# UnofficialJuliaMirrorSnapshots/TrajectoryOptimization.jl-c79d492b-0548-5874-b488-5a62c1d9d0ca

Hardware: AMD Instinct MI355X
Metric: iLQR iterations/sec (batched trajectories), quadrotor n=13 m=4 N=101 (higher is better)
Workload: dtype f64

## Files before the change

### trajectoryoptimization.jl-c79d492b-0548-5874-b488-5a62c1d9d0ca_amd/csrc/tog_host_plan.hpp

```cpp
#pragma once
#include <algorithm>
#include <cmath>
#include <cstddef>
#include <cstring>
#include <type_traits>
#include <vector>

namespace tog_plan {

template <int... Vs, class F>
inline void pick(int v, F&& f) {
  (void)((v == Vs && (f(std::integral_constant<int, Vs>{}), true)) || ...);
}

inline bool chol_upper(const double* A, int n, double* U) {
  for (int i = 0; i < n * n; i++) U[i] = 0.0;
  for (int j = 0; j < n; j++) {
    double s = A[j + n * j];
    for (int k = 0; k < j; k++) s -= U[k + n * j] * U[k + n * j];
    if (!(s > 0.0)) return false;
    const double ujj = std::sqrt(s);
    U[j + n * j] = ujj;
    for (int c = j + 1; c < n; c++) {
      double t = A[j + n * c];
      for (int k = 0; k < j; k++) t -= U[k + n * j] * U[k + n * c];
      U[j + n * c] = t / ujj;
    }
  }
  return true;
}

struct CostPlan {
  int nc_in = 0, kst = 0, nk = 0;
  int n = 0, m = 0;
  std::vector<double> kc;
  std::vector<double> cQf;
  bool sqrt_ok = false;
  int diag_cost = 0;
  const double* Q(int k) const { return kc.data() + (size_t)k * kst; }
  const double* R(int k) const { return Q(k) + n * n; }
  const double* H(int k) const { return R(k) + m * m; }
  const double* q(int k) const { return H(k) + m * n; }
  const double* r(int k) const { return q(k) + n; }
  double c(int k) const { return Q(k)[nc_in - 1]; }
  const double* cQ(int k) const { return Q(k) + nc_in; }
  const double* cR(int k) const { return cQ(k) + n * n; }
};

inline CostPlan plan_costs(int n, int m, int N, double dt, const double* Q, const double* R, const double* H,
                           const double* q, const double* r, double c, const double* stage_costs,
                           const double* Qf) {
  CostPlan p;
  p.n = n;
  p.m = m;
  p.nc_in = n * n + m * m + m * n + n + m + 1;
  p.kst = 2 * n * n + 2 * m * m + m * n + n + m + 1;
  p.nk = stage_costs ? N - 1 : 1;
  const int nc_in = p.nc_in, nk = p.nk;
  p.kc.assign((size_t)nk * p.kst, 0.0);
  for (int k = 0; k < nk; k++) {
    double* o = p.kc.data() + (size_t)k * p.kst;
    if (stage_costs) {
      memcpy(o, stage_costs + (size_t)k * nc_in, sizeof(double) * nc_in);
    } else {
      memcpy(o, Q, sizeof(double) * n * n);
      memcpy(o + n * n, R, sizeof(double) * m * m);
      memcpy(o + n * n + m * m, H, sizeof(double) * m * n);
      memcpy(o + n * n + m * m + m * n, q, sizeof(double) * n);
      memcpy(o + n * n + m * m + m * n + n, r, sizeof(double) * m);
      o[nc_in - 1] = c;
    }
  }
  auto kcQ = [&](int k) { return p.kc.data() + (size_t)k * p.kst + nc_in; };
  auto kcR = [&](int k) { return kcQ(k) + n * n; };
  p.cQf.assign((size_t)n * n, 0.0);
  bool ok = chol_upper(Qf, n, p.cQf.data());
  std::vector<double> Qdt((size_t)n * n), Rdt((size_t)m * m);
  for (int k = 0; k < nk; k++) {
    for (int i = 0; i < n * n; i++) Qdt[i] = p.Q(k)[i] * dt;
    for (int i = 0; i < m * m; i++) Rdt[i] = p.R(k)[i] * dt;
    ok = chol_upper(Qdt.data(), n, kcQ(k)) && chol_upper(Rdt.data(), m, kcR(k)) && ok;
  }
  p.sqrt_ok = ok;
  bool diag = true;
  for (int j = 0; j < n; j++)
    for (int i = 0; i < n; i++)
      if (i != j && Qf[i + n * j] != 0.0) diag = false;
  for (int k = 0; k < nk; k++) {
    for (int j = 0; j < n; j++)
      for (int i = 0; i < n; i++)
        if (i != j && p.Q(k)[i + n * j] != 0.0) diag = false;
    for (int j = 0; j < m; j++)
      for (int i = 0; i < m; i++)
        if (i != j && p.R(k)[i + m * j] != 0.0) diag = false;
    for (int i = 0; i < m * n; i++)
// ... 44 lines not shown
```

### trajectoryoptimization.jl-c79d492b-0548-5874-b488-5a62c1d9d0ca_amd/csrc/tog_kernels.hpp

```cpp
#pragma once

#include "tog_device.hpp"
#include <string.h>

namespace tog {

constexpr int PCAP = 72;
template <class M>
__host__ __device__ constexpr int pcap_of() { return PCAP; }
constexpr int WAVE = 64;

__device__ __forceinline__ long long traj_of_slot(const DevBuffers& Bf, long long i, long long B) {
  if (Bf.act_list) return i < (long long)*Bf.act_count ? (long long)Bf.act_list[i] : -1;
  return i < B ? i : -1;
}
__device__ __forceinline__ long long slot_count(const DevBuffers& Bf, long long B) {
  return Bf.act_list ? (long long)*Bf.act_count : B;
}

__device__ __forceinline__ void wsync() { __syncthreads(); }

template <class M>
__host__ __device__ constexpr int cand_w() {
  return M::n + M::m;
// ... 2482 lines not shown
  const long long b = (phase == 2) ? (long long)list[t] : traj_of_slot(Bf, t, P->B);
  if (!Bf.st[b].active) return;
  if (phase == 1 && !ls_decided_within(P->o, Bf, b, Bf.nc, bookkeeping ? Bf.st[b].J : Jprev_in[b], Bf.st[b].dV0,
                                       Bf.st[b].dV1, hi))
    return;
  constexpr int n = M::n, m = M::m;
  const tog_options& o = P->o;
  const bool al = (mode == TOG_MODE_AL);
  const int N = P->N, NC = Bf.nc;
  TrajState s = Bf.st[b];
  const double J_prev = bookkeeping ? s.J : Jprev_in[b];
  double J = INFINITY, z = -1.0, expected = 0.0, alpha_last = 0.0;
  int trials = 0, state = 0;
  for (int jj = 0;; jj++) {
    if (!((z <= o.line_search_lower_bound || z > o.line_search_upper_bound) && J >= J_prev)) {
      state = 1;
      break;
    }
    if (jj > o.iterations_linesearch) {
      state = 2;
      break;
    }
    trials++;
    const double aj = ldexp(1.0, -jj);
    bool ok;
    double Jj;
    if (jj < NC) {
      ok = Bf.lsok[b * NC + jj] != 0;
      Jj = Bf.lsJ[b * NC + jj];
    } else {
      ok = rollout_cost<M, INTEG, 0>(P, Bf, b, aj, al, Jj, nullptr, RT);
    }
    if (!ok) continue;
    J = Jj;
    expected = -aj * (s.dV0 + aj * s.dV1);
    z = (expected > 0.0) ? (J_prev - J) / expected : -1.0;
    alpha_last = aj;
  }
  double grad = 0.0;
  bool copied = false;
  if (state == 2) {
    const double* X = Bf.X + (size_t)b * N * n;
    const double* U = Bf.U + (size_t)b * (N - 1) * m;
    if (!bookkeeping) {
      double* Xb = Bf.Xb + (size_t)b * N * n;
      double* Ub = Bf.Ub + (size_t)b * (N - 1) * m;
      for (int i = 0; i < N * n; i++) Xb[i] = X[i];
      for (int i = 0; i < (N - 1) * m; i++) Ub[i] = U[i];
    }
    J = traj_cost<M>(P, Bf, b, X, U, al, al ? Bf.C + (size_t)b * N * P->pmax : nullptr);
    z = 0.0;
    expected = 0.0;
    alpha_last = 0.0;
    reg_increase(P, s);
    s.rho += o.bp_reg_fp;
    grad = traj_gradient<M>(P, Bf, b, al);
    copied = true;
  } else if (!bookkeeping) {
    double Jw;
    rollout_cost<M, INTEG, 1>(P, Bf, b, alpha_last, al, Jw, nullptr, RT);
  } else if (!(J > o.max_cost_value)) {
    double Jw;
    rollout_cost<M, INTEG, 2>(P, Bf, b, alpha_last, al, Jw, &grad, RT);
    copied = true;
  }
  if (bookkeeping && copied && state != 2 && o.gradient_type != 0) grad = traj_gradient<M>(P, Bf, b, al);
  s.alpha = alpha_last;
  s.z = z;
  s.expected = expected;
  s.ls_trials = trials;
  if (J > J_prev) s.flags |= TOG_TRAJ_COST_INCREASED;
  if (Jout) Jout[b] = J;
  if (bookkeeping) {
    if (s.flags & TOG_TRAJ_COST_INCREASED) {
      s.active = 0;
    } else {
      step_bookkeeping<M>(P, Bf, b, s, J, copied, grad, mode);
    }
  }
  Bf.st[b] = s;
}


template <class M>
__global__ void __launch_bounds__(256) k_ls_decide(const DevProblem* __restrict__ P, DevBuffers Bf, int hi,
                                                   int bookkeeping, const double* __restrict__ Jprev_in,
                                                   const int* __restrict__ in_list, const int* __restrict__ in_count,
                                                   int* __restrict__ out_list, int* __restrict__ out_count, int pend) {
  const long long t = (long long)blockIdx.x * blockDim.x + threadIdx.x;
  const long long nb = in_list ? (long long)*in_count : slot_count(Bf, P->B);
  bool und = false;
  long long b = 0;
  if (t < nb) {
    b = in_list ? (long long)in_list[t] : traj_of_slot(Bf, t, P->B);
    TrajState* st = Bf.st + b;
    if (st->active) {
      const tog_options& o = P->o;
      const int NC = Bf.nc;
      const double J_prev = bookkeeping ? st->J : Jprev_in[b];
      const double dV0 = st->dV0, dV1 = st->dV1;
      if (pend) hi = (st->ls_pend + hi < NC) ? st->ls_pend + hi : NC;
      double J = INFINITY, z = -1.0, expected = 0.0, alpha_last = 0.0;
      int trials = 0, state = 0, win = -1;
      for (int jj = 0;; jj++) {
        if (!((z <= o.line_search_lower_bound || z > o.line_search_upper_bound) && J >= J_prev)) {
          state = 1;
          break;
        }
        if (jj > o.iterations_linesearch) {
          state = 2;
          break;
        }
        if (jj >= hi) break;
        trials++;
        if (!Bf.lsok[b * NC + jj]) continue;
        const double aj = ldexp(1.0, -jj);
        J = Bf.lsJ[b * NC + jj];
        expected = -aj * (dV0 + aj * dV1);
        z = (expected > 0.0) ? (J_prev - J) / expected : -1.0;
        alpha_last = aj;
        win = jj;
      }
      if (state == 0) {
        und = true;
        if (pend) {
          st->ls_pend = hi;
          Bf.ls_win[b] = -9;
        }
      } else {
        st->ls_pend = 0;
        if (state == 2) {
          win = -2;
          z = 0.0;
          expected = 0.0;
          alpha_last = 0.0;
          if (Bf.ls_fb) Bf.ls_fb[atomicAdd(Bf.ls_count + 2, 1)] = (int)b;
        } else if (win < 0) {
          win = -3;
        }
        st->alpha = alpha_last;
        st->z = z;
        st->expected = expected;
        st->ls_trials = trials;
        Bf.ls_win[b] = win;
        Bf.ls_Jw[b] = J;
      }
    }
  }
  if (!out_list || pend) return;
  const unsigned long long mask = __ballot(und);
  if (mask == 0) return;
  const int lane = threadIdx.x & (WAVE - 1);
  const int leader = __ffsll((long long)mask) - 1;
  int base = 0;
  if (lane == leader) base = atomicAdd(out_count, __popcll(mask));
  base = __shfl(base, leader);
  if (und) out_list[base + __popcll(mask & ((1ull << lane) - 1))] = (int)b;
}

template <class M>
__global__ void __launch_bounds__(256) k_ls_apply(const DevProblem* __restrict__ P, DevBuffers Bf, int bookkeeping) {
  constexpr int n = M::n, m = M::m, Q = cand_q<M>();
  const int N = P->N;
  const unsigned per = (unsigned)N * Q;
  const unsigned long long t = (unsigned long long)blockIdx.x * blockDim.x + threadIdx.x;
  const long long slot = (long long)(t / per);
  if (slot >= slot_count(Bf, P->B)) return;
  const long long b = traj_of_slot(Bf, slot, P->B);
  const unsigned r = (unsigned)(t - (unsigned long long)slot * per);
  const int k = (int)(r / Q), q = (int)(r - (unsigned)k * Q);
  if (!Bf.st[b].active) return;
  const int w = Bf.ls_win[b];
  if (w < 0) return;
  if (bookkeeping && Bf.ls_Jw[b] > P->o.max_cost_value) return;
  const int ncp = Bf.ncp;
  const double* tb = Bf.cand + (size_t)b * per * ncp * 4;
  const double* src = tb + ((size_t)r * ncp + w) * 4;
  double v[4];
#pragma unroll
  for (int e = 0; e < 4; e++) v[e] = src[e];
  double* Xd = (bookkeeping ? Bf.X : Bf.Xb) + ((size_t)b * N + k) * n;
  double* Ud = (bookkeeping ? Bf.U : Bf.Ub) + ((size_t)b * (N - 1) + k) * m;
#pragma unroll
  for (int e = 0; e < 4; e++) {
    const int c = 4 * q + e;
    if (c < m) {
      if (k < N - 1) Ud[c] = v[e];
    } else if (c < m + n) {
      Xd[c - m] = (k == 0) ? Bf.x0[(size_t)b * n + c - m] : v[e];
    }
  }
  if (bookkeeping && q == 0 && k < N - 1) {
    const double* dk = Bf.d + ((size_t)b * (N - 1) + k) * m;
    double mx = -INFINITY;
#pragma unroll
    for (int i = 0; i < m; i++) {
      const double ui = (i < 4) ? v[i] : tb[cand_at(k, i, Q, ncp) + (size_t)w * 4];
      const double vv = fabs(dk[i]) / (fabs(ui) + 1.0);
      if (vv > mx || isnan(vv)) mx = vv;
    }
    Bf.gk[(size_t)b * N + k] = mx;
  }
}

template <class M, int INTEG>
__device__ __noinline__ void replay_cost(const DevProblem* __restrict__ P, const DevBuffers& Bf, long long b,
                                         double alpha, bool al, int bookkeeping, double max_cost, double J,
                                         double& grad, bool& copied, const RowTables& RT) {
  double Jw;
  if (!bookkeeping) {
    rollout_cost<M, INTEG, 1>(P, Bf, b, alpha, al, Jw, nullptr, RT);
  } else if (!(J > max_cost)) {
    rollout_cost<M, INTEG, 2>(P, Bf, b, alpha, al, Jw, &grad, RT);
    copied = true;
  }
}

template <class M>
__global__ void __launch_bounds__(64) k_ls_fallback(const DevProblem* __restrict__ P, DevBuffers Bf, int al,
                                                    const int* __restrict__ list, const int* __restrict__ count) {
  if ((int)blockIdx.x >= *count) return;
  extern __shared__ double fb_lds[];
  constexpr int n = M::n, m = M::m;
  const int N = P->N, pmax = P->pmax;
  const long long b = list[blockIdx.x];
  const int lane = threadIdx.x;
  double* sk = fb_lds;
  double* ak = fb_lds + N;
  int* hk = reinterpret_cast<int*>(fb_lds + 2 * N);
  const double* X = Bf.X + (size_t)b * N * n;
  const double* U = Bf.U + (size_t)b * (N - 1) * m;
  const double* d = Bf.d + (size_t)b * (N - 1) * m;
  double* C = Bf.C + (size_t)b * N * pmax;
  const double* lam = Bf.lam + (size_t)b * N * pmax;
  const double* mu = Bf.mu + (size_t)b * N * pmax;
  for (int k = lane; k < N; k += WAVE) {
    const double* x = X + (size_t)k * n;
    const double* u = (k < N - 1) ? U + (size_t)k * m : nullptr;
    sk[k] = (k < N - 1) ? stage_cost_m<M>(P, b, k, x, u) : terminal_cost_m<M>(P, b, x);
    const int cnt = al ? knot_count(P, k) : 0;
    const cptr<ConRow> rows = knot_rows(P, k);
    double lc = 0.0, cIc = 0.0;
    for (int i = 0; i < cnt; i++) {
      const size_t q = (size_t)k * pmax + i;
      const ConRow r = traj_row(P, b, load_row(rows + i));
      const double c = row_value_m<M>(r, x, u);
      const double l = lam[q];
      const bool a = row_inequality<(ModelTraits<M>::slack > 0)>(r) ? ((c >= 0.0) || (l > 0.0)) : true;
      const double w = a ? mu[q] : 0.0;
      lc = fma(l, c, lc);
      cIc = fma(c * w, c, cIc);
      C[q] = c;
    }
    ak[k] = lc + 0.5 * cIc;
    hk[k] = cnt;
    if (k < N - 1) {
      double mx = -INFINITY;
#pragma unroll
      for (int i = 0; i < m; i++) {
        const double v = fabs(d[(size_t)k * m + i]) / (fabs(u[i]) + 1.0);
        if (v > mx || isnan(v)) mx = v;
      }
      Bf.gk[(size_t)b * N + k] = mx;
    }
  }
  __syncthreads();
  if (lane != 0) return;
  double J = 0.0, Jc = 0.0;
  for (int k = 0; k < N - 1; k++) J += sk[k];
  J += sk[N - 1];
  for (int k = 0; k < N; k++)
    if (hk[k]) Jc += ak[k];
  Bf.ls_Jw[b] = al ? J + Jc : J;
}

template <class M, int INTEG>
__global__ void __launch_bounds__(64) k_ls_book(const DevProblem* __restrict__ P, DevBuffers Bf, int mode,
                                                int bookkeeping, const double* Jprev_in, double* Jout) {
  const long long t = (long long)blockIdx.x * blockDim.x + threadIdx.x;
  extern __shared__ double rt_lds[];
  const RowTables RT =
      (mode == TOG_MODE_AL && Bf.rows_lds > 0) ? block_row_tables(P, rt_lds) : global_row_tables(P);
  if (t >= slot_count(Bf, P->B)) return;
  const long long b = traj_of_slot(Bf, t, P->B);
  if (!Bf.st[b].active) return;
  constexpr int n = M::n, m = M::m;
  const tog_options& o = P->o;
  const bool al = (mode == TOG_MODE_AL);
  const int N = P->N;
  const int win = Bf.ls_win[b];
  if (win == -9) return;
  TrajState s = Bf.st[b];
  double J = Bf.ls_Jw[b];
  const double J_prev = bookkeeping ? s.J : Jprev_in[b];
  double grad = 0.0;
  bool copied = false;
  if (win == -2) {
    if (!bookkeeping) {
      const double* X = Bf.X + (size_t)b * N * n;
      const double* U = Bf.U + (size_t)b * (N - 1) * m;
      double* Xb = Bf.Xb + (size_t)b * N * n;
      double* Ub = Bf.Ub + (size_t)b * (N - 1) * m;
      for (int i = 0; i < N * n; i++) Xb[i] = X[i];
      for (int i = 0; i < (N - 1) * m; i++) Ub[i] = U[i];
    }
    reg_increase(P, s);
    s.rho += o.bp_reg_fp;
    if (o.gradient_type == 0) {
      const double* g = Bf.gk + (size_t)b * N;
      double gsum = 0.0;
      for (int k = 0; k < N - 1; k++) gsum += g[k];
      grad = gsum / N;
    } else {
      grad = traj_gradient<M>(P, Bf, b, al);
    }
    copied = true;
  } else if (win == -3) {
    replay_cost<M, INTEG>(P, Bf, b, s.alpha, al, bookkeeping, o.max_cost_value, J, grad, copied, RT);
  } else if (bookkeeping && !(J > o.max_cost_value)) {
    const double* g = Bf.gk + (size_t)b * N;
    double gsum = 0.0;
    for (int k = 0; k < N - 1; k++) gsum += g[k];
    grad = gsum / N;
    copied = true;
  }
  if (bookkeeping && copied && win != -2 && o.gradient_type != 0) grad = traj_gradient<M>(P, Bf, b, al);
  if (J > J_prev) s.flags |= TOG_TRAJ_COST_INCREASED;
  if (Jout) Jout[b] = J;
  (void)copied;
  if (bookkeeping) {
    if (s.flags & TOG_TRAJ_COST_INCREASED) {
      s.active = 0;
    } else if (inner_bookkeeping(P, Bf, b, s, J, grad, mode)) {
      Bf.ls_done[atomicAdd(Bf.ls_count + 1, 1)] = (int)b;
    }
  }
  Bf.st[b] = s;
}

template <class M>
__global__ void __launch_bounds__(64) k_al_outer(const DevProblem* __restrict__ P, DevBuffers Bf, int mode,
                                                 const int* __restrict__ list, const int* __restrict__ count) {
  if ((int)blockIdx.x >= *count) return;
  extern __shared__ double alo_lds[];
  constexpr int n = M::n, m = M::m;
  constexpr bool SL = ModelTraits<M>::slack > 0;
  const int N = P->N, pmax = P->pmax;
  const tog_options& o = P->o;
  const long long b = list[blockIdx.x];
  const int lane = threadIdx.x;
  double* sk = alo_lds;
  double* ak = alo_lds + N;
  int* hk = reinterpret_cast<int*>(alo_lds + 2 * N);
  const double* X = Bf.X + (size_t)b * N * n;
  const double* U = Bf.U + (size_t)b * (N - 1) * m;
  double* C = Bf.C + (size_t)b * N * pmax;
  double* lam = Bf.lam + (size_t)b * N * pmax;
  double* mu = Bf.mu + (size_t)b * N * pmax;
  double mumax = 0.0, cmax = 0.0;
  for (int k = lane; k < N; k += WAVE) {
    const double* x = X + (size_t)k * n;
    const double* u = (k < N - 1) ? U + (size_t)k * m : nullptr;
    sk[k] = (k < N - 1) ? stage_cost_m<M>(P, b, k, x, u) : terminal_cost_m<M>(P, b, x);
    const int cnt = knot_count(P, k);
    const cptr<ConRow> rows = knot_rows(P, k);
    double lc = 0.0, cIc = 0.0, e = 0.0, im = -INFINITY;
    int ni = 0;
    for (int i = 0; i < cnt; i++) {
      const size_t q = (size_t)k * pmax + i;
      const ConRow r = traj_row(P, b, load_row(rows + i));
      const double c = row_value_m<M>(r, x, u);
      C[q] = c;
      const bool ineq = row_inequality<SL>(r);
      double l = lam[q] + mu[q] * c;
      l = tog_jlmax(o.dual_min, tog_jlmin(o.dual_max, l));
      if (ineq) l = tog_jlmax(0.0, l);
      const double mn = fmax(0.0, fmin(o.penalty_max, o.penalty_scaling * mu[q]));
      lam[q] = l;
      mu[q] = mn;
      mumax = fmax(mumax, mn);
      if (ineq) {
        ni++;
        im = tog_jlmax(im, c);
      } else {
        e = tog_jlmax(e, fabs(c));
      }
      const bool a = ineq ? ((c >= 0.0) || (l > 0.0)) : true;
      const double w = a ? mn : 0.0;
      lc = fma(l, c, lc);
      cIc = fma(c * w, c, cIc);
    }
    if (cnt) {
      cmax = tog_jlmax(e, cmax);
      if (ni > 0) cmax = tog_jlmax(tog_jlmax(0.0, im), cmax);
    }
    ak[k] = lc + 0.5 * cIc;
    hk[k] = cnt;
  }
#pragma unroll
  for (int off = 32; off >= 1; off >>= 1) {
    mumax = fmax(mumax, __shfl_xor(mumax, off));
    cmax = tog_jlmax(cmax, __shfl_xor(cmax, off));
  }
  __syncthreads();
  if (lane != 0) return;
  TrajState s = Bf.st[b];
  const bool conv = (o.kickout_max_penalty && mumax == o.penalty_max) || (cmax < o.constraint_tolerance);
  double Jnext = 0.0;
  if (!conv && s.al_iter < o.al_iterations) {
    double J = 0.0, Jc = 0.0;
    for (int k = 0; k < N - 1; k++) J += sk[k];
    J += sk[N - 1];
    for (int k = 0; k < N; k++)
      if (hk[k]) Jc += ak[k];
    Jnext = J + Jc;
  }
  const double gnext = (Bf.hist_in && !conv && s.al_iter < o.al_iterations) ? traj_gradient<M>(P, Bf, b, true) : 0.0;
  al_outer_finish(P, Bf, b, s, mumax, cmax, s.J, Jnext, gnext, mode);
  Bf.st[b] = s;
}

}
#include "tog_bwd_team.hpp"
#include "tog_bwd_quad.hpp"
#include "tog_pn.hpp"
namespace tog {

template <class M, int INTEG>
__global__ void __launch_bounds__(64) k_slack_controls(const DevProblem* __restrict__ P, DevBuffers Bf) {
  using Mb = typename ModelTraits<M>::Base;
  constexpr int n = M::n, m = M::m;
  const long long b = (long long)blockIdx.x * blockDim.x + threadIdx.x;
  if (b >= P->B) return;
  const int N = P->N;
  const double* X = Bf.X + (size_t)b * N * n;
  double* U = Bf.U + (size_t)b * (N - 1) * m;
  double x[n], xn[n];
#pragma unroll
  for (int i = 0; i < n; i++) x[i] = Bf.x0[(size_t)b * n + i];
  for (int k = 0; k < N - 1; k++) {
    double* u = U + (size_t)k * m;
    discrete_step<Mb, INTEG>(xn, x, u, P->dt);
#pragma unroll
    for (int i = 0; i < n; i++) {
      const double sl = X[(size_t)(k + 1) * n + i] - xn[i];
      u[Mb::m + i] = sl;
      x[i] = xn[i] + sl;
    }
  }
}

__device__ inline bool dev_chol_upper(double* U, const double* A, int n) {
  for (int i = 0; i < n * n; i++) U[i] = 0.0;
  for (int j = 0; j < n; j++) {
    double s = A[j + n * j];
    for (int k = 0; k < j; k++) s -= U[k + n * j] * U[k + n * j];
    if (!(s > 0.0)) return false;
    const double ujj = sqrt(s);
    U[j + n * j] = ujj;
    for (int c = j + 1; c < n; c++) {
      double t = A[j + n * c];
      for (int k = 0; k < j; k++) t -= U[k + n * j] * U[k + n * c];
      U[j + n * c] = t / ujj;
    }
  }
  return true;
}

__device__ inline void dev_qr_R(double* R, double* Pm, int rows, int cols) {
  const int kmax = rows < cols ? rows : cols;
  for (int j = 0; j < kmax; j++) {
    const double alpha = Pm[j + rows * j];
    double acc[4] = {0.0, 0.0, 0.0, 0.0};
    for (int i = j + 1; i < rows; i++) acc[(i - j - 1) & 3] = fma(Pm[i + rows * j], Pm[i + rows * j], acc[(i - j - 1) & 3]);
    const double ss = (acc[0] + acc[1]) + (acc[2] + acc[3]);
    if (ss == 0.0) continue;
    const double beta = -copysign(sqrt(fma(alpha, alpha, ss)), alpha);
    const double vd = alpha - beta;
    const double rd = 1.0 / (beta * vd);
    Pm[j + rows * j] = beta;
    for (int c = j + 1; c < cols; c++) {
      double a4[4] = {0.0, 0.0, 0.0, 0.0};
      for (int i = j + 1; i < rows; i++) a4[(i - j - 1) & 3] = fma(Pm[i + rows * j], Pm[i + rows * c], a4[(i - j - 1) & 3]);
      const double p = fma(vd, Pm[j + rows * c], (a4[0] + a4[1]) + (a4[2] + a4[3])) * rd;
      Pm[j + rows * c] = fma(vd, p, Pm[j + rows * c]);
      for (int i = j + 1; i < rows; i++) Pm[i + rows * c] = fma(Pm[i + rows * j], p, Pm[i + rows * c]);
    }
  }
  for (int j = 0; j < cols; j++)
    for (int i = 0; i < cols; i++) R[i + cols * j] = (i <= j && i < rows) ? Pm[i + rows * j] : 0.0;
}

template <class M>
__global__ void __launch_bounds__(64) k_cost_expansion(const DevProblem* __restrict__ P, DevBuffers Bf, int sq,
                                                       int al, int* fail) {
  constexpr int n = M::n, m = M::m, NQ = nq_of<M>(), PC = pcap_of<M>(), W = n > m ? n : m;
  const long long t = (long long)blockIdx.x * blockDim.x + threadIdx.x;
  const int N = P->N;
  if (t >= P->B * (long long)N) return;
  const int k = (int)(t % N);
  const long long b = t / N;
  const bool term = (k == N - 1);
// ... 126 lines not shown
```

### trajectoryoptimization.jl-c79d492b-0548-5874-b488-5a62c1d9d0ca_amd/csrc/tog_launch.hpp

```cpp
#pragma once

#include "tog_kernels.hpp"
#include "tog_host_plan.hpp"

namespace tog {

using tog_plan::pick;

inline int ali_backward(int al, int tv) { return (al ? 1 : 0) | (tv ? 2 : 0); }
inline int ali_expand(int al, int tv) { return (al ? 1 : 0) | ((tv & 2) ? 2 : 0); }

struct StreamPair {
  hipStream_t st2;
  hipEvent_t fork, join;
};

struct ModelOps {
  int n, m;
  int slack;
  int pcap;
  int has_con;
  int min_time;
  long long jws_per_lane;
  void (*slack_controls)(const DevProblem*, const DevBuffers&, long long B, int integ, hipStream_t);
// ... 41 lines not shown
    }
    if (integ == TOG_RK4) {
      f(std::integral_constant<int, TOG_RK4>{});
    } else if (integ == TOG_MIDPOINT) {
      f(std::integral_constant<int, TOG_MIDPOINT>{});
    } else if (integ == TOG_RK3_IMPLICIT || integ == TOG_MIDPOINT_IMPLICIT) {
      if constexpr (ModelTraits<M>::implicit_ok) {
        if (integ == TOG_RK3_IMPLICIT)
          f(std::integral_constant<int, TOG_RK3_IMPLICIT>{});
        else
          f(std::integral_constant<int, TOG_MIDPOINT_IMPLICIT>{});
      }
    } else {
      f(std::integral_constant<int, TOG_RK3>{});
    }
  }
  static void init(const DevProblem* P, const DevBuffers& Bf, long long B, int integ, int mode, hipStream_t st) {
    with_integ(integ, [&](auto ic) {
      constexpr int I = decltype(ic)::value;
      hipLaunchKernelGGL((k_init<M, I>), dim3(grid(B, 64)), dim3(64), 0, st, P, Bf, mode);
    });
  }
  static void refill(const DevProblem* P, const DevBuffers& Bf, int count, int N, int integ, int mode, const int* list,
                     const double* x0, const double* U, const double* X, hipStream_t st) {
    if (count <= 0) return;
    const unsigned sm = (unsigned)(N * (2 * sizeof(double) + sizeof(int)));
    with_integ(integ, [&](auto ic) {
      constexpr int I = decltype(ic)::value;
      hipLaunchKernelGGL((k_refill<M, I>), dim3((unsigned)count), dim3(64), sm, st, P, Bf, mode, list, count, x0, U, X);
    });
  }
  static void rollout_open(const DevProblem* P, const DevBuffers& Bf, long long B, int integ, hipStream_t st) {
    with_integ(integ, [&](auto ic) {
      constexpr int I = decltype(ic)::value;
      hipLaunchKernelGGL((k_rollout_open<M, I>), dim3(grid(B, 64)), dim3(64), 0, st, P, Bf);
    });
  }
  static void jacobian(const DevProblem* P, const DevBuffers& Bf, long long B, int N, int integ, hipStream_t st) {
    if constexpr (ModelTraits<M>::min_time) {
      using Mc = typename ModelTraits<M>::Core;
      constexpr int NCHT = (Mc::n + Mc::m + 1 + JW - 1) / JW;
      const long long total = B * (long long)(N - 1) * NCHT;
      with_integ(integ, [&](auto ic) {
        constexpr int I = decltype(ic)::value;
        hipLaunchKernelGGL((k_jacobian_mt<M, I, JW>), dim3(grid(total, 256)), dim3(256), 0, st, P, Bf, total);
      });
    } else if (Mb::id == TOG_MODEL_KUKA && integ == TOG_RK3 && Bf.jws) {
      if constexpr (Mb::id == TOG_MODEL_KUKA && ModelTraits<M>::explicit_ok) {
        const long long total = B * (long long)(N - 1);
        hipLaunchKernelGGL((k_kuka_points<M>), dim3(grid(total, 64)), dim3(64), 0, st, P, Bf, total);
        hipLaunchKernelGGL((k_kuka_sjac<M, 0>), dim3(grid(total * 21, 256)), dim3(256), 0, st, P, Bf, total);
        hipLaunchKernelGGL((k_kuka_sjac<M, 1>), dim3(grid(total * 21, 256)), dim3(256), 0, st, P, Bf, total);
        hipLaunchKernelGGL((k_kuka_chain<M>), dim3((unsigned)total), dim3(64), 0, st, P, Bf, total);
      }
    } else {
      constexpr int NCH = (Mb::n + Mb::m + JW - 1) / JW;
      const long long total = B * (long long)(N - 1) * NCH;
      with_integ(integ, [&](auto ic) {
        constexpr int I = decltype(ic)::value;
        hipLaunchKernelGGL((k_jacobian<M, I, JW>), dim3(grid(total, 256)), dim3(256), 0, st, P, Bf, total);
      });
    }
  }
  static void backward(const DevProblem* P, const DevBuffers& Bf, long long B, int sq, int al, int flags, int team,
                       hipStream_t st) {
    if constexpr (M::m <= M::n && M::n + 1 <= 16 && !ModelTraits<M>::min_time) {
    if (team) {
      constexpr int TPW = TeamCfg<M>::TPW;
      const dim3 g((unsigned)((B + TPW - 1) / TPW)), blk(64);
      DevBuffers Bl = Bf;
      Bl.bwd_stride = Bf.bwd_stride2[sq ? 1 : 0];
      Bl.bwd_shmem = Bf.bwd_shmem2[sq ? 1 : 0];
      const unsigned sm = (unsigned)Bl.bwd_shmem;
      const int ali = ali_backward(al, Bf.tv);
      auto launch = [&](auto wpe_c) {
        pick<0, 1>(sq ? 1 : 0, [&](auto sq_c) {
          pick<0, 1, 2, 3>(ali, [&](auto ali_c) {
            hipLaunchKernelGGL((k_bwd_team<M, decltype(sq_c)::value, decltype(ali_c)::value, decltype(wpe_c)::value>),
                               g, blk, sm, st, P, Bl, flags);
          });
        });
      };
      const char* tk = getenv("TOG_BWD_TAIL");
      const bool quad = !(tk && !strcmp(tk, "team"));
      if (Bf.tail && sq && TeamCfg<M>::TEAM == 16 && quad) {
        if constexpr (TeamCfg<M>::TEAM == 16) {
          pick<0, 1, 2, 3>(ali, [&](auto ali_c) {
            hipLaunchKernelGGL((k_bwd_quad<M, decltype(ali_c)::value>), dim3((unsigned)B), dim3(256), 0, st, P, Bf,
                               flags);
          });
        }
      } else if (Bf.tail || (B + TPW - 1) / TPW <= Bf.simds) {
        launch(std::integral_constant<int, 1>{});
      } else {
        launch(std::integral_constant<int, TOG_BWD_WAVES>{});
      }
      return;
    }
    }
    pick<0, 1>(sq ? 1 : 0, [&](auto sq_c) {
      pick<0, 1>(al ? 1 : 0, [&](auto al_c) {
        hipLaunchKernelGGL((k_backward<M, decltype(sq_c)::value, decltype(al_c)::value>), dim3((unsigned)B), dim3(64),
                           0, st, P, Bf, flags);
      });
    });
  }
  static void expand(const DevProblem* P, const DevBuffers& Bf, long long B, int N, int pmax, int sq, int al,
                     hipStream_t st) {
    if constexpr (M::m <= M::n && M::n + 1 <= 16 && !ModelTraits<M>::min_time) {
      constexpr int TPW = TeamCfg<M>::TPW;
      const unsigned sm = (unsigned)(sizeof(double) * TPW * expand_team_stride<M>(pmax));
      int mode = 0;
      const int ali = ali_expand(al, Bf.tv);
      if constexpr (M::m <= 4 && TeamCfg<M>::TEAM == 16) {
        const char* eq = getenv("TOG_EXPAND_QUAD");
        if (sq && !(eq && eq[0] == '0')) {
          const long long qteams = B * (long long)(N - 1);
          pick<0, 1, 2, 3>(ali, [&](auto ali_c) {
            hipLaunchKernelGGL((k_expand_u<M, decltype(ali_c)::value>), dim3((unsigned)((qteams + 15) / 16)), dim3(64),
                               0, st, P, Bf);
          });
          mode = (al && Bf.dense_stage_knots) ? 1 : 2;
        }
      }
      const long long teams = (mode == 2) ? B : B * (long long)N;
      const dim3 g((unsigned)((teams + TPW - 1) / TPW)), blk(64);
      pick<0, 1>(sq ? 1 : 0, [&](auto sq_c) {
        pick<0, 1, 2, 3>(ali, [&](auto ali_c) {
          hipLaunchKernelGGL((k_expand_team<M, decltype(sq_c)::value, decltype(ali_c)::value>), g, blk, sm, st, P, Bf,
                             mode);
        });
      });
    }
  }
  template <int INTEG>
  static void spec(const DevProblem* P, const DevBuffers& Bf, long long B, int mode, int lo, int cnt, const int* list,
                   const int* count, hipStream_t st) {
    const bool diag = Bf.cost_diag && !(Bf.tv & 2);
    if (Bf.tail && Bf.cand && Bf.spec_tail2_shmem > 0 && diag && !list && cnt <= SPEC_LANES) {
      hipLaunchKernelGGL((k_ls_spec_tail2<M, INTEG, 1>), dim3((unsigned)B), dim3(3 * WAVE),
                         (unsigned)Bf.spec_tail2_shmem, st, P, Bf, mode, lo, cnt);
      return;
    }
    if (Bf.tail && Bf.cand && Bf.spec_tail_shmem > 0 && diag && !list && cnt <= WAVE) {
      hipLaunchKernelGGL((k_ls_spec_tail<M, INTEG, 1>), dim3((unsigned)B), dim3(WAVE), (unsigned)Bf.spec_tail_shmem, st,
                         P, Bf, mode, lo, cnt);
      return;
    }
    const unsigned gs = grid(B * (long long)cnt, 256);
    const unsigned rb = (mode == TOG_MODE_AL) ? (unsigned)Bf.rows_lds : 0u;
    pick<0, 1>(Bf.cand ? 1 : 0, [&](auto cand_c) {
      pick<0, 1>(rb ? 1 : 0, [&](auto lrt_c) {
        pick<0, 1>(diag ? 1 : 0, [&](auto diag_c) {
          constexpr bool CAND = decltype(cand_c)::value != 0, LRT = decltype(lrt_c)::value != 0;
          constexpr int DC = CAND ? decltype(diag_c)::value : 0;
          if constexpr (M::n * M::m > 64)
            hipLaunchKernelGGL((k_ls_spec_w1<M, INTEG, CAND, LRT, DC>), dim3(grid(B * (long long)cnt, 64)), dim3(64),
                               LRT ? rb : 0u, st, P, Bf, mode, lo, cnt, list, count);
          else
            hipLaunchKernelGGL((k_ls_spec<M, INTEG, CAND, LRT, DC>), dim3(gs), dim3(256), LRT ? rb : 0u, st, P, Bf,
                               mode, lo, cnt, list, count);
        });
      });
    });
  }
  template <int INTEG>
  static void forward_cand(const DevProblem* P, const DevBuffers& Bf, long long B, int mode, int bk, const double* Jp,
                           double* Jo, hipStream_t st) {
    const int F = Bf.ls_first;
    (void)hipMemsetAsync(Bf.ls_count, 0, sizeof(int) * LS_COUNT_SLOTS, st);
    if (F >= Bf.nc) {
      spec<INTEG>(P, Bf, B, mode, 0, Bf.nc, nullptr, nullptr, st);
      hipLaunchKernelGGL((k_ls_decide<M>), dim3(grid(B, 256)), dim3(256), 0, st, P, Bf, Bf.nc, bk, Jp, nullptr,
                         nullptr, nullptr, nullptr, 0);
    } else if (bk && Bf.ls_pend_ok) {
      spec<INTEG>(P, Bf, B, mode, 0, F, nullptr, nullptr, st);
      hipLaunchKernelGGL((k_ls_decide<M>), dim3(grid(B, 256)), dim3(256), 0, st, P, Bf, F, bk, Jp, nullptr, nullptr,
                         nullptr, nullptr, 1);
    } else {
      spec<INTEG>(P, Bf, B, mode, 0, F, nullptr, nullptr, st);
      hipLaunchKernelGGL((k_ls_decide<M>), dim3(grid(B, 256)), dim3(256), 0, st, P, Bf, F, bk, Jp, nullptr, nullptr,
                         Bf.ls_list, Bf.ls_count, 0);
      spec<INTEG>(P, Bf, B, mode, F, Bf.nc - F, Bf.ls_list, Bf.ls_count, st);
      hipLaunchKernelGGL((k_ls_decide<M>), dim3(grid(B, 256)), dim3(256), 0, st, P, Bf, Bf.nc, bk, Jp, Bf.ls_list,
                         Bf.ls_count, nullptr, nullptr, 0);
    }
    const long long tot = B * (long long)Bf.nknots * cand_q<M>();
    hipLaunchKernelGGL((k_ls_apply<M>), dim3(grid(tot, 256)), dim3(256), 0, st, P, Bf, bk);
    hipLaunchKernelGGL((k_ls_fallback<M>), dim3((unsigned)B), dim3(64),
                       (unsigned)(Bf.nknots * (2 * sizeof(double) + sizeof(int))), st, P, Bf,
                       (int)(mode == TOG_MODE_AL), Bf.ls_fb, Bf.ls_count + 2);
    hipLaunchKernelGGL((k_ls_book<M, INTEG>), dim3(grid(B, 64)), dim3(64), (unsigned)Bf.rows_lds, st, P, Bf, mode,
                       bk, Jp, Jo);
    if (bk && mode == TOG_MODE_AL) {
      const unsigned sm = (unsigned)(Bf.nknots * (2 * sizeof(double) + sizeof(int)));
      hipLaunchKernelGGL((k_al_outer<M>), dim3((unsigned)B), dim3(64), sm, st, P, Bf, mode, Bf.ls_done,
                         Bf.ls_count + 1);
    }
  }
  template <int INTEG>
  static void commit(const DevProblem* P, const DevBuffers& Bf, long long B, int mode, int bk, const double* Jp,
                     double* Jo, int phase, int hi, const int* list, const int* count, hipStream_t st) {
    hipLaunchKernelGGL((k_ls_commit<M, INTEG>), dim3(grid(B, 64)), dim3(64), (unsigned)Bf.rows_lds, st, P, Bf, mode,
                       bk, Jp, Jo, phase, hi, list, count);
  }
  template <int INTEG>
  static void forward_i(const DevProblem* P, const DevBuffers& Bf, long long B, int mode, int bk, const double* Jp,
                        double* Jo, hipStream_t st, const StreamPair* sp) {
    if (Bf.cand) {
      forward_cand<INTEG>(P, Bf, B, mode, bk, Jp, Jo, st);
      return;
    }
    (void)hipMemsetAsync(Bf.ls_count, 0, sizeof(int) * LS_COUNT_SLOTS, st);
    if (sp && LS_MAX_ROUNDS == 2 && Bf.nc > LS_FIRST) {
      spec<INTEG>(P, Bf, B, mode, 0, LS_FIRST, nullptr, nullptr, st);
      int* list = Bf.ls_list + (size_t)B;
      int* count = Bf.ls_count + 1;
      hipLaunchKernelGGL((k_ls_compact<M>), dim3(grid(B, 256)), dim3(256), 0, st, P, Bf, LS_FIRST, bk, Jp, nullptr,
                         nullptr, list, count);
      (void)hipEventRecord(sp->fork, st);
      (void)hipStreamWaitEvent(sp->st2, sp->fork, 0);
      commit<INTEG>(P, Bf, B, mode, bk, Jp, Jo, 1, LS_FIRST, nullptr, nullptr, sp->st2);
      spec<INTEG>(P, Bf, B, mode, LS_FIRST, Bf.nc - LS_FIRST, list, count, st);
      commit<INTEG>(P, Bf, B, mode, bk, Jp, Jo, 2, LS_FIRST, list, count, st);
      (void)hipEventRecord(sp->join, sp->st2);
      (void)hipStreamWaitEvent(st, sp->join, 0);
      return;
    }
    int lo = 0, round = 0;
    const int* list = nullptr;
    const int* count = nullptr;
    while (lo < Bf.nc) {
      const int hi = (round + 1 < LS_MAX_ROUNDS) ? (lo == 0 ? LS_FIRST : 2 * lo) : Bf.nc;
      const int cnt = (hi < Bf.nc ? hi : Bf.nc) - lo;
      if (round > 0) {
        int* out = Bf.ls_list + (size_t)(round & 1) * B;
        hipLaunchKernelGGL((k_ls_compact<M>), dim3(grid(B, 256)), dim3(256), 0, st, P, Bf, lo, bk, Jp,
                           list, count, out, Bf.ls_count + round);
        list = out;
        count = Bf.ls_count + round;
      }
      spec<INTEG>(P, Bf, B, mode, lo, cnt, list, count, st);
      lo += cnt;
      round++;
    }
    commit<INTEG>(P, Bf, B, mode, bk, Jp, Jo, 0, 0, nullptr, nullptr, st);
  }
  static void forward(const DevProblem* P, const DevBuffers& Bf, long long B, int integ, int mode, int bk,
                      const double* Jp, double* Jo, hipStream_t st, const StreamPair* sp) {
    with_integ(integ, [&](auto ic) { forward_i<decltype(ic)::value>(P, Bf, B, mode, bk, Jp, Jo, st, sp); });
  }
  static void cost(const DevProblem* P, const DevBuffers& Bf, long long B, int al, int bar, double* J,
// ... 106 lines not shown
```

Before: 88670.

## Fuse line-search decide/apply/fallback/bookkeeping/AL-outer into one tail kernel

Factors the line-search decide, apply, fallback, bookkeeping and AL outer-update kernels into device helpers. It adds a single per-trajectory kernel, k_ls_finish, that runs them in sequence when in the tail phase with bookkeeping and all candidates evaluated. This replaces a memset plus several kernel launches with atomics-based lists, cutting launch overhead when few trajectories remain. The tail backward kernel choice (quad vs team) is now picked by a heuristic on batch width versus CU count instead of always using quad. The cost is serial single-thread sections inside one block and one block per trajectory, including inactive ones.

Result: faster. 91980 (median of 6 runs) (+3.7%).

```diff
diff --git a/trajectoryoptimization.jl-c79d492b-0548-5874-b488-5a62c1d9d0ca_amd/csrc/tog_host_plan.hpp b/trajectoryoptimization.jl-c79d492b-0548-5874-b488-5a62c1d9d0ca_amd/csrc/tog_host_plan.hpp
--- a/trajectoryoptimization.jl-c79d492b-0548-5874-b488-5a62c1d9d0ca_amd/csrc/tog_host_plan.hpp
+++ b/trajectoryoptimization.jl-c79d492b-0548-5874-b488-5a62c1d9d0ca_amd/csrc/tog_host_plan.hpp
@@ -11,6 +11,12 @@
 template <int... Vs, class F>
 inline void pick(int v, F&& f) {
   (void)((v == Vs && (f(std::integral_constant<int, Vs>{}), true)) || ...);
+}
+
+enum TailBackward { TAIL_BWD_TEAM = 0, TAIL_BWD_QUAD = 1 };
+constexpr long long TAIL_QUAD_ROUNDS = 1;
+inline TailBackward tail_backward(long long width, int cus) {
+  return (cus > 0 && width <= TAIL_QUAD_ROUNDS * (long long)cus) ? TAIL_BWD_QUAD : TAIL_BWD_TEAM;
 }
 
 inline bool chol_upper(const double* A, int n, double* U) {
diff --git a/trajectoryoptimization.jl-c79d492b-0548-5874-b488-5a62c1d9d0ca_amd/csrc/tog_kernels.hpp b/trajectoryoptimization.jl-c79d492b-0548-5874-b488-5a62c1d9d0ca_amd/csrc/tog_kernels.hpp
--- a/trajectoryoptimization.jl-c79d492b-0548-5874-b488-5a62c1d9d0ca_amd/csrc/tog_kernels.hpp
+++ b/trajectoryoptimization.jl-c79d492b-0548-5874-b488-5a62c1d9d0ca_amd/csrc/tog_kernels.hpp
@@ -2588,6 +2588,60 @@
 }
 
 
+__device__ inline int ls_decide_traj(const DevProblem* __restrict__ P, const DevBuffers& Bf, long long b, int hi,
+                                     int bookkeeping, const double* __restrict__ Jprev_in, int pend) {
+  TrajState* st = Bf.st + b;
+  const tog_options& o = P->o;
+  const int NC = Bf.nc;
+  const double J_prev = bookkeeping ? st->J : Jprev_in[b];
+  const double dV0 = st->dV0, dV1 = st->dV1;
+  if (pend) hi = (st->ls_pend + hi < NC) ? st->ls_pend + hi : NC;
+  double J = INFINITY, z = -1.0, expected = 0.0, alpha_last = 0.0;
+  int trials = 0, state = 0, win = -1;
+  for (int jj = 0;; jj++) {
+    if (!((z <= o.line_search_lower_bound || z > o.line_search_upper_bound) && J >= J_prev)) {
+      state = 1;
+      break;
+    }
+    if (jj > o.iterations_linesearch) {
+      state = 2;
+      break;
+    }
+    if (jj >= hi) break;
+    trials++;
+    if (!Bf.lsok[b * NC + jj]) continue;
+    const double aj = ldexp(1.0, -jj);
+    J = Bf.lsJ[b * NC + jj];
+    expected = -aj * (dV0 + aj * dV1);
+    z = (expected > 0.0) ? (J_prev - J) / expected : -1.0;
+    alpha_last = aj;
+    win = jj;
+  }
+  if (state == 0) {
+    if (pend) {
+      st->ls_pend = hi;
+      Bf.ls_win[b] = -9;
+    }
+    return 0;
+  }
+  st->ls_pend = 0;
+  if (state == 2) {
+    win = -2;
+    z = 0.0;
+    expected = 0.0;
+    alpha_last = 0.0;
+  } else if (win < 0) {
+    win = -3;
+  }
+  st->alpha = alpha_last;
+  st->z = z;
+  st->expected = expected;
+  st->ls_trials = trials;
+  Bf.ls_win[b] = win;
+  Bf.ls_Jw[b] = J;
+  return state;
+}
+
 template <class M>
 __global__ void __launch_bounds__(256) k_ls_decide(const DevProblem* __restrict__ P, DevBuffers Bf, int hi,
                                                    int bookkeeping, const double* __restrict__ Jprev_in,
@@ -2599,58 +2653,10 @@
   long long b = 0;
   if (t < nb) {
     b = in_list ? (long long)in_list[t] : traj_of_slot(Bf, t, P->B);
-    TrajState* st = Bf.st + b;
-    if (st->active) {
-      const tog_options& o = P->o;
-      const int NC = Bf.nc;
-      const double J_prev = bookkeeping ? st->J : Jprev_in[b];
-      const double dV0 = st->dV0, dV1 = st->dV1;
-      if (pend) hi = (st->ls_pend + hi < NC) ? st->ls_pend + hi : NC;
-      double J = INFINITY, z = -1.0, expected = 0.0, alpha_last = 0.0;
-      int trials = 0, state = 0, win = -1;
-      for (int jj = 0;; jj++) {
-        if (!((z <= o.line_search_lower_bound || z > o.line_search_upper_bound) && J >= J_prev)) {
-          state = 1;
-          break;
-        }
-        if (jj > o.iterations_linesearch) {
-          state = 2;
-          break;
-        }
-        if (jj >= hi) break;
-        trials++;
-        if (!Bf.lsok[b * NC + jj]) continue;
-        const double aj = ldexp(1.0, -jj);
-        J = Bf.lsJ[b * NC + jj];
-        expected = -aj * (dV0 + aj * dV1);
-        z = (expected > 0.0) ? (J_prev - J) / expected : -1.0;
-        alpha_last = aj;
-        win = jj;
-      }
-      if (state == 0) {
-        und = true;
-        if (pend) {
-          st->ls_pend = hi;
-          Bf.ls_win[b] = -9;
-        }
-      } else {
-        st->ls_pend = 0;
-        if (state == 2) {
-          win = -2;
-          z = 0.0;
-          expected = 0.0;
-          alpha_last = 0.0;
-          if (Bf.ls_fb) Bf.ls_fb[atomicAdd(Bf.ls_count + 2, 1)] = (int)b;
-        } else if (win < 0) {
-          win = -3;
-        }
-        st->alpha = alpha_last;
-        st->z = z;
-        st->expected = expected;
-        st->ls_trials = trials;
-        Bf.ls_win[b] = win;
-        Bf.ls_Jw[b] = J;
-      }
+    if (Bf.st[b].active) {
+      const int state = ls_decide_traj(P, Bf, b, hi, bookkeeping, Jprev_in, pend);
+      und = (state == 0);
+      if (state == 2 && Bf.ls_fb) Bf.ls_fb[atomicAdd(Bf.ls_count + 2, 1)] = (int)b;
     }
   }
   if (!out_list || pend) return;
@@ -2665,20 +2671,12 @@
 }
 
 template <class M>
-__global__ void __launch_bounds__(256) k_ls_apply(const DevProblem* __restrict__ P, DevBuffers Bf, int bookkeeping) {
+__device__ __forceinline__ void ls_apply_quad(const DevProblem* __restrict__ P, const DevBuffers& Bf, long long b,
+                                              unsigned r, int w, int bookkeeping) {
   constexpr int n = M::n, m = M::m, Q = cand_q<M>();
   const int N = P->N;
   const unsigned per = (unsigned)N * Q;
-  const unsigned long long t = (unsigned long long)blockIdx.x * blockDim.x + threadIdx.x;
-  const long long slot = (long long)(t / per);
-  if (slot >= slot_count(Bf, P->B)) return;
-  const long long b = traj_of_slot(Bf, slot, P->B);
-  const unsigned r = (unsigned)(t - (unsigned long long)slot * per);
   const int k = (int)(r / Q), q = (int)(r - (unsigned)k * Q);
-  if (!Bf.st[b].active) return;
-  const int w = Bf.ls_win[b];
-  if (w < 0) return;
-  if (bookkeeping && Bf.ls_Jw[b] > P->o.max_cost_value) return;
   const int ncp = Bf.ncp;
   const double* tb = Bf.cand + (size_t)b * per * ncp * 4;
   const double* src = tb + ((size_t)r * ncp + w) * 4;
@@ -2707,6 +2705,21 @@
     }
     Bf.gk[(size_t)b * N + k] = mx;
   }
+}
+
+template <class M>
+__global__ void __launch_bounds__(256) k_ls_apply(const DevProblem* __restrict__ P, DevBuffers Bf, int bookkeeping) {
+  const unsigned per = (unsigned)P->N * cand_q<M>();
+  const unsigned long long t = (unsigned long long)blockIdx.x * blockDim.x + threadIdx.x;
+  const long long slot = (long long)(t / per);
+  if (slot >= slot_count(Bf, P->B)) return;
+  const long long b = traj_of_slot(Bf, slot, P->B);
+  const unsigned r = (unsigned)(t - (unsigned long long)slot * per);
+  if (!Bf.st[b].active) return;
+  const int w = Bf.ls_win[b];
+  if (w < 0) return;
+  if (bookkeeping && Bf.ls_Jw[b] > P->o.max_cost_value) return;
+  ls_apply_quad<M>(P, Bf, b, r, w, bookkeeping);
 }
 
 template <class M, int INTEG>
@@ -2723,14 +2736,10 @@
 }
 
 template <class M>
-__global__ void __launch_bounds__(64) k_ls_fallback(const DevProblem* __restrict__ P, DevBuffers Bf, int al,
-                                                    const int* __restrict__ list, const int* __restrict__ count) {
-  if ((int)blockIdx.x >= *count) return;
-  extern __shared__ double fb_lds[];
+__device__ __forceinline__ void ls_fallback_knots(const DevProblem* __restrict__ P, const DevBuffers& Bf, int al,
+                                                  long long b, int lane, double* fb_lds) {
   constexpr int n = M::n, m = M::m;
   const int N = P->N, pmax = P->pmax;
-  const long long b = list[blockIdx.x];
-  const int lane = threadIdx.x;
   double* sk = fb_lds;
   double* ak = fb_lds + N;
   int* hk = reinterpret_cast<int*>(fb_lds + 2 * N);
@@ -2770,8 +2779,13 @@
       Bf.gk[(size_t)b * N + k] = mx;
     }
   }
-  __syncthreads();
-  if (lane != 0) return;
+}
+__device__ inline void ls_fallback_sum(const DevProblem* __restrict__ P, const DevBuffers& Bf, int al, long long b,
+                                       const double* fb_lds) {
+  const int N = P->N;
+  const double* sk = fb_lds;
+  const double* ak = fb_lds + N;
+  const int* hk = reinterpret_cast<const int*>(fb_lds + 2 * N);
   double J = 0.0, Jc = 0.0;
   for (int k = 0; k < N - 1; k++) J += sk[k];
   J += sk[N - 1];
@@ -2780,22 +2794,26 @@
   Bf.ls_Jw[b] = al ? J + Jc : J;
 }
 
+template <class M>
+__global__ void __launch_bounds__(64) k_ls_fallback(const DevProblem* __restrict__ P, DevBuffers Bf, int al,
+                                                    const int* __restrict__ list, const int* __restrict__ count) {
+  if ((int)blockIdx.x >= *count) return;
+  extern __shared__ double fb_lds[];
+  const long long b = list[blockIdx.x];
+  ls_fallback_knots<M>(P, Bf, al, b, (int)threadIdx.x, fb_lds);
+  __syncthreads();
+  if (threadIdx.x == 0) ls_fallback_sum(P, Bf, al, b, fb_lds);
+}
+
 template <class M, int INTEG>
-__global__ void __launch_bounds__(64) k_ls_book(const DevProblem* __restrict__ P, DevBuffers Bf, int mode,
-                                                int bookkeeping, const double* Jprev_in, double* Jout) {
-  const long long t = (long long)blockIdx.x * blockDim.x + threadIdx.x;
-  extern __shared__ double rt_lds[];
-  const RowTables RT =
-      (mode == TOG_MODE_AL && Bf.rows_lds > 0) ? block_row_tables(P, rt_lds) : global_row_tables(P);
-  if (t >= slot_count(Bf, P->B)) return;
-  const long long b = traj_of_slot(Bf, t, P->B);
-  if (!Bf.st[b].active) return;
+__device__ __forceinline__ bool ls_book_traj(const DevProblem* __restrict__ P, const DevBuffers& Bf, long long b,
+                                             int win, int mode, int bookkeeping, const double* Jprev_in,
+                                             double* Jout, const RowTables& RT) {
   constexpr int n = M::n, m = M::m;
   const tog_options& o = P->o;
   const bool al = (mode == TOG_MODE_AL);
   const int N = P->N;
-  const int win = Bf.ls_win[b];
-  if (win == -9) return;
+  bool outer = false;
   TrajState s = Bf.st[b];
   double J = Bf.ls_Jw[b];
   const double J_prev = bookkeeping ? s.J : Jprev_in[b];
@@ -2837,24 +2855,37 @@
   if (bookkeeping) {
     if (s.flags & TOG_TRAJ_COST_INCREASED) {
       s.active = 0;
-    } else if (inner_bookkeeping(P, Bf, b, s, J, grad, mode)) {
-      Bf.ls_done[atomicAdd(Bf.ls_count + 1, 1)] = (int)b;
+    } else {
+      outer = inner_bookkeeping(P, Bf, b, s, J, grad, mode);
     }
   }
   Bf.st[b] = s;
+  return outer;
+}
+
+template <class M, int INTEG>
+__global__ void __launch_bounds__(64) k_ls_book(const DevProblem* __restrict__ P, DevBuffers Bf, int mode,
+                                                int bookkeeping, const double* Jprev_in, double* Jout) {
+  const long long t = (long long)blockIdx.x * blockDim.x + threadIdx.x;
+  extern __shared__ double rt_lds[];
+  const RowTables RT =
+      (mode == TOG_MODE_AL && Bf.rows_lds > 0) ? block_row_tables(P, rt_lds) : global_row_tables(P);
+  if (t >= slot_count(Bf, P->B)) return;
+  const long long b = traj_of_slot(Bf, t, P->B);
+  if (!Bf.st[b].active) return;
+  const int win = Bf.ls_win[b];
+  if (win == -9) return;
+  if (ls_book_traj<M, INTEG>(P, Bf, b, win, mode, bookkeeping, Jprev_in, Jout, RT))
+    Bf.ls_done[atomicAdd(Bf.ls_count + 1, 1)] = (int)b;
 }
 
 template <class M>
-__global__ void __launch_bounds__(64) k_al_outer(const DevProblem* __restrict__ P, DevBuffers Bf, int mode,
-                                                 const int* __restrict__ list, const int* __restrict__ count) {
-  if ((int)blockIdx.x >= *count) return;
-  extern __shared__ double alo_lds[];
+__device__ __forceinline__ void al_outer_knots(const DevProblem* __restrict__ P, const DevBuffers& Bf, long long b,
+                                               int lane, double* alo_lds, double& mumax_out, double& cmax_out) {
   constexpr int n = M::n, m = M::m;
   constexpr bool SL = ModelTraits<M>::slack > 0;
   const int N = P->N, pmax = P->pmax;
   const tog_options& o = P->o;
-  const long long b = list[blockIdx.x];
-  const int lane = threadIdx.x;
   double* sk = alo_lds;
   double* ak = alo_lds + N;
   int* hk = reinterpret_cast<int*>(alo_lds + 2 * N);
@@ -2908,8 +2939,17 @@
     mumax = fmax(mumax, __shfl_xor(mumax, off));
     cmax = tog_jlmax(cmax, __shfl_xor(cmax, off));
   }
-  __syncthreads();
-  if (lane != 0) return;
+  mumax_out = mumax;
+  cmax_out = cmax;
+}
+template <class M>
+__device__ __forceinline__ void al_outer_sum(const DevProblem* __restrict__ P, const DevBuffers& Bf, int mode,
+                                             long long b, const double* alo_lds, double mumax, double cmax) {
+  const int N = P->N;
+  const tog_options& o = P->o;
+  const double* sk = alo_lds;
+  const double* ak = alo_lds + N;
+  const int* hk = reinterpret_cast<const int*>(alo_lds + 2 * N);
   TrajState s = Bf.st[b];
   const bool conv = (o.kickout_max_penalty && mumax == o.penalty_max) || (cmax < o.constraint_tolerance);
   double Jnext = 0.0;
@@ -2924,6 +2964,60 @@
   const double gnext = (Bf.hist_in && !conv && s.al_iter < o.al_iterations) ? traj_gradient<M>(P, Bf, b, true) : 0.0;
   al_outer_finish(P, Bf, b, s, mumax, cmax, s.J, Jnext, gnext, mode);
   Bf.st[b] = s;
+}
+
+template <class M>
+__global__ void __launch_bounds__(64) k_al_outer(const DevProblem* __restrict__ P, DevBuffers Bf, int mode,
+                                                 const int* __restrict__ list, const int* __restrict__ count) {
+  if ((int)blockIdx.x >= *count) return;
+  extern __shared__ double alo_lds[];
+  const long long b = list[blockIdx.x];
+  double mumax, cmax;
+  al_outer_knots<M>(P, Bf, b, (int)threadIdx.x, alo_lds, mumax, cmax);
+  __syncthreads();
+  if (threadIdx.x == 0) al_outer_sum<M>(P, Bf, mode, b, alo_lds, mumax, cmax);
+}
+
+constexpr int LS_FINISH_THREADS = 256;
+template <class M, int INTEG>
+__global__ void __launch_bounds__(LS_FINISH_THREADS) k_ls_finish(const DevProblem* __restrict__ P, DevBuffers Bf,
+                                                                 int mode, const double* Jprev_in, double* Jout) {
+  extern __shared__ double fin_lds[];
+  __shared__ int v_win, v_fb, v_outer;
+  __shared__ double v_J;
+  const long long b = traj_of_slot(Bf, blockIdx.x, P->B);
+  if (b < 0) return;
+  if (!Bf.st[b].active) return;
+  const int tid = threadIdx.x;
+  const bool al = (mode == TOG_MODE_AL);
+  if (tid == 0) {
+    v_fb = (ls_decide_traj(P, Bf, b, Bf.nc, 1, Jprev_in, 0) == 2);
+    v_win = Bf.ls_win[b];
+    v_J = Bf.ls_Jw[b];
+    v_outer = 0;
+  }
+  __syncthreads();
+  const int win = v_win;
+  if (win == -9) return;
+  if (win >= 0 && !(v_J > P->o.max_cost_value)) {
+    const unsigned per = (unsigned)P->N * cand_q<M>();
+    for (unsigned r = tid; r < per; r += LS_FINISH_THREADS) ls_apply_quad<M>(P, Bf, b, r, win, 1);
+  }
+  if (v_fb) {
+    if (tid < WAVE) ls_fallback_knots<M>(P, Bf, al ? 1 : 0, b, tid, fin_lds);
+    __syncthreads();
+    if (tid == 0) ls_fallback_sum(P, Bf, al ? 1 : 0, b, fin_lds);
+  }
+  const RowTables RT =
+      (win == -3 && al && Bf.rows_lds > 0) ? block_row_tables(P, fin_lds) : global_row_tables(P);
+  __syncthreads();
+  if (tid == 0) v_outer = ls_book_traj<M, INTEG>(P, Bf, b, win, mode, 1, Jprev_in, Jout, RT) ? 1 : 0;
+  __syncthreads();
+  if (!v_outer) return;
+  double mumax = 0.0, cmax = 0.0;
+  if (tid < WAVE) al_outer_knots<M>(P, Bf, b, tid, fin_lds, mumax, cmax);
+  __syncthreads();
+  if (tid == 0) al_outer_sum<M>(P, Bf, mode, b, fin_lds, mumax, cmax);
 }
 
 }
diff --git a/trajectoryoptimization.jl-c79d492b-0548-5874-b488-5a62c1d9d0ca_amd/csrc/tog_launch.hpp b/trajectoryoptimization.jl-c79d492b-0548-5874-b488-5a62c1d9d0ca_amd/csrc/tog_launch.hpp
--- a/trajectoryoptimization.jl-c79d492b-0548-5874-b488-5a62c1d9d0ca_amd/csrc/tog_launch.hpp
+++ b/trajectoryoptimization.jl-c79d492b-0548-5874-b488-5a62c1d9d0ca_amd/csrc/tog_launch.hpp
@@ -147,7 +147,9 @@
         });
       };
       const char* tk = getenv("TOG_BWD_TAIL");
-      const bool quad = !(tk && !strcmp(tk, "team"));
+      const bool quad = (tk && !strcmp(tk, "team"))   ? false
+                        : (tk && !strcmp(tk, "quad")) ? true
+                                                      : tog_plan::tail_backward(B, Bf.simds / 4) == tog_plan::TAIL_BWD_QUAD;
       if (Bf.tail && sq && TeamCfg<M>::TEAM == 16 && quad) {
         if constexpr (TeamCfg<M>::TEAM == 16) {
           pick<0, 1, 2, 3>(ali, [&](auto ali_c) {
@@ -233,6 +235,17 @@
   static void forward_cand(const DevProblem* P, const DevBuffers& Bf, long long B, int mode, int bk, const double* Jp,
                            double* Jo, hipStream_t st) {
     const int F = Bf.ls_first;
+    const unsigned knots_lds = (unsigned)(Bf.nknots * (2 * sizeof(double) + sizeof(int)));
+    if (F >= Bf.nc && bk && Bf.tail) {
+      const char* lf = getenv("TOG_LS_FINISH");
+      if (!(lf && !strcmp(lf, "split"))) {
+        spec<INTEG>(P, Bf, B, mode, 0, Bf.nc, nullptr, nullptr, st);
+        const unsigned rows = (mode == TOG_MODE_AL) ? (unsigned)Bf.rows_lds : 0u;
+        hipLaunchKernelGGL((k_ls_finish<M, INTEG>), dim3((unsigned)B), dim3(LS_FINISH_THREADS),
+                           knots_lds > rows ? knots_lds : rows, st, P, Bf, mode, Jp, Jo);
+        return;
+      }
+    }
     (void)hipMemsetAsync(Bf.ls_count, 0, sizeof(int) * LS_COUNT_SLOTS, st);
     if (F >= Bf.nc) {
       spec<INTEG>(P, Bf, B, mode, 0, Bf.nc, nullptr, nullptr, st);
```
